# hgpeterson/nuPGCM

Measured on AMD Instinct MI355X. Metric: timesteps/sec (evolve!+invert! loop; inversion SpMV GB/s in 'roofline'), higher is better.
Workload: dtype f64 arithmetic; fp32-STORED Krylov basis and fp32 gather-layout copy of the SpMV input (the library's default at rtol >= 1e-7; products, sums, x += V y and the restart residual are fp64 - the all-fp64 figure is `fp64_basis`); 1 GPU; bowl3D_h0.02: example parameters of examples/bowl_mixing.jl (eps=0.2, alpha=1/2, mu_rho=1, N2=2, BDF2 dt=0.001), full evolve!+invert! timestep loop; tets=526720, nu=2052199, np=98592, nb=707204, nnz_A=126821881, node_block_storage=True, full_nodes=658911, surface_nodes=37733, gmres_memory=20, gmres_itmax=0, initial_guess=x_{n-1} (the reference's warm start), all_solved=True, preconditioner=Diagonal(scalar=73847.66715287707), parallelism=1 GPU

## Files before the change

nupgcm_amd/csrc/gmres.hip:

```cpp
#include <algorithm>
#include <chrono>
#include <cmath>
#include <cstdlib>
#include <type_traits>

#include <hip/hip_ext.h>

#include "common.h"
#include "spmv_device.h"
#include "spmv_window.h"

namespace npg {

constexpr int kKB = 512;
constexpr int kKP = kPartStride;
constexpr int kNS = kKB / kKP;
constexpr int kMaxG = 768;
constexpr int kMaxI = kMaxG / kNS;
constexpr int kNormSlot = kKP - 1;
constexpr int kMaxRows = 2048;

struct Snap {
    double eps, rnorm0, rnorm, beta, zeta;
    int iter, inner, done, npass, first, nreorth, pad0, pad1;
};

struct GParams {
    double atol, rtol, eta2, btol;
    long long itmax;
};

struct GDev {
    CsrDev A;
    const TileDesc *tile_ptr;
    int ntiles, n, mem;
    int nt_int;
    const WTileDesc *wt_ptr;
    WinDev W;
    int nwt, nwt_int, wl;
    int word;
    int wpre;
    int pkind;
    double pscalar;
    const double *pdiag;
    const double *b;
    double *x, *Vi, *w, *wt;
    double *P1, *P2, *PR;
    int G1, G2, GP1, GP2;
    int GR;
    int split;
    int64_t ldv;
    float *Vf;
    int pyth;
    int lazy2;
    int rev;
    GatherMap xg;
    const int32_t *gslot;
    int fast;
    const double *Q1, *Q2, *QR;
    int nQ1, nQ2, nQR;
    Snap *C, *T;
    double *c, *s, *z, *R, *hcol1, *wnorm2;
    double *hist;
    int hist_cap;
    const GParams *prm;
};

__device__ __forceinline__ void sym_givens(double a, double b, double &c, double &s, double &rho) {
    if (b == 0.0) {
        c = (a == 0.0) ? 1.0 : copysign(1.0, a);
        s = 0.0;
        rho = fabs(a);
    } else if (a == 0.0) {
        c = 0.0;
        s = copysign(1.0, b);
        rho = fabs(b);
    } else if (fabs(b) > fabs(a)) {
        const double t = a / b;
        s = copysign(1.0, b) / sqrt(1.0 + t * t);
        c = s * t;
        rho = b / s;
    } else {
        const double t = b / a;
        c = copysign(1.0, a) / sqrt(1.0 + t * t);
        s = c * t;
        rho = a / c;
    }
}

struct KShared {
    double red[kKP];
    double h[kKP], h2[kKP], cc[kKP], ss[kKP], y[kKP];
    Snap T;
    double rho, zcol;
    int fin;
    int reorth;
};

__device__ __forceinline__ void store_partial_row(double acc, double *tmp, double *part) {
    __syncthreads();
    tmp[threadIdx.x] = acc;
    __syncthreads();
    if (threadIdx.x < kKP) {
        double s = 0.0;
#pragma unroll
        for (int sl = 0; sl < kNS; ++sl) s += tmp[sl * kKP + threadIdx.x];
        part[(size_t)blockIdx.x * kKP + threadIdx.x] = s;
    }
}

__device__ void finalize_column(const GDev &d, int colj, KShared &sh, double *tmp) {
    const int t32 = threadIdx.x & (kKP - 1);
    const double h1 = d.hcol1[colj * kKP + t32];
    const double cv = d.c[t32], sv = d.s[t32];
    const Snap prev = d.T[colj];
    const double wnorm2 = d.wnorm2[colj];
    const double q1 = group_sum_dpp<kKP>(t32 <= colj ? h1 * h1 : 0.0);
    const double n2f = wnorm2 - q1;
    const bool need2 = !d.pyth && (!d.lazy2 || !(n2f >= fmax(d.prm->eta2, 1e-4) * wnorm2));
    if (need2) reduce_partials<kNS, kMaxI>(d.Q2, d.nQ2, kKP, tmp, sh.red);
    if (threadIdx.x < kKP) {
        sh.h[threadIdx.x] = h1;
        sh.h2[threadIdx.x] = (need2 && !d.fast && (int)threadIdx.x <= colj) ? sh.red[threadIdx.x] : 0.0;
        sh.cc[threadIdx.x] = cv;
        sh.ss[threadIdx.x] = sv;
    }
    __syncthreads();
    if (threadIdx.x == 0) {
        Snap t = prev;
        sh.fin = (t.done == 0) ? 1 : 0;
        sh.reorth = 0;
        if (t.done == 0) {
            double n2;
            if (d.pyth) {
                n2 = fmax(n2f, 0.0);
                if (n2f < 1e-4 * wnorm2) {
                    t.pad0 += 1;
                    t.done = 5;
                    sh.fin = 0;
                }
            } else if (!need2) {
                n2 = fmax(n2f, 0.0);
            } else {
// ... 84 lines not shown
    double acc = 0.0;
    if (c.done == 0) {
        TileDesc nd = d.tile_ptr[blockIdx.x < (unsigned)d.ntiles ? blockIdx.x : 0];
        for (int t = blockIdx.x; t < d.ntiles; t += gridDim.x) {
            const TileDesc td = nd;
            if (t + (int)gridDim.x < d.ntiles) nd = d.tile_ptr[t + gridDim.x];
            const int r0 = td.r0, r1 = td.r0 + td.nrows;
            spmv_tile<kKB, L, PlainX, kTileNnz, 4, NoProf, false, false, N9>(d.A, PlainX{d.x}, td, tl, sw);
            const int r = threadIdx.x;
            if (r < r1 - r0) {
                const int row = r0 + r;
                const double res = precond_row(d, row) * (d.b[row] - sw[r]);
                d.wt[row] = res;
                if (d.xg.p) d.xg.p[d.xg.pos(row)] = (float)res;
                acc += res * res;
            }
        }
    }
    acc = group_sum_dpp<kKP>(acc);
    store_partial_row((threadIdx.x & (kKP - 1)) == 0 ? acc : 0.0, tmp, d.PR);
}

template <int L, bool FUSED, int XG = 0, bool N9 = false, int WL = 0, bool ORD = true>
__global__ void __launch_bounds__(kKB, FUSED ? 4 : 6) k_gmres_arnoldi(GDev d, int j, int t0, int t1) {
    static_assert(WL == 0 || (XG == 1 && !N9 && !FUSED), "windowed tiles serve the gather-layout instance of the split organisation");
    __shared__ KShared sh;
    __shared__ TileLds tl;
    __shared__ double sw[kTileRows];
    double *tmp = tl.prod;
    using TD = std::conditional_t<WL != 0, WTileDesc, TileDesc>;
    const TD *__restrict__ tiles;
    if constexpr (WL != 0) tiles = d.wt_ptr; else tiles = d.tile_ptr;
    TD nd = tiles[t0 + (int)blockIdx.x < t1 ? t0 + (int)blockIdx.x : 0];
    WinPre pre;
    bool have = false;
    if constexpr (WL != 0) {
        if (d.wpre && t0 + (int)blockIdx.x < t1 && nd.nw) {
            win_first<kKB>(d.W, PaddedX{d.xg}, nd, pre);
            have = true;
        }
    }
    if (j == 0) {
        const Snap c = *d.C;
        reduce_partials<kNS, kMaxI>(d.QR, d.nQR, 1, tmp, sh.red);
        if (threadIdx.x == 0) {
            Snap t = c;
            if (t.done == 0) {
                const double beta = sqrt(sh.red[0]);
                if (t.first) {
                    t.rnorm0 = beta;
                    t.rnorm = beta;
                    t.eps = d.prm->atol + d.prm->rtol * beta;
                    t.first = 0;
                    if (blockIdx.x == 0) d.hist[0] = beta;
                    if (beta == 0.0) t.done = 4;
                }
                t.beta = beta;
                t.zeta = beta;
                t.npass += 1;
            }
            t.inner = 0;
            sh.T = t;
            sh.reorth = 0;
            if (blockIdx.x == 0) d.T[0] = t;
        }
        __syncthreads();
    } else {
        finalize_column(d, j - 1, sh, tmp);
    }
    const Snap T = sh.T;
    if (T.done != 0) return;

    const int k = threadIdx.x & (kKP - 1), slot = threadIdx.x >> 5;
    const double inv_beta = 1.0 / T.beta;
    const bool ro = XG == 0 && sh.reorth != 0;
    const double h2k = (ro && k < j) ? sh.h2[k] : 0.0;
    double acc = 0.0;
    for (int t = t0 + blockIdx.x; t < t1; t += gridDim.x) {
        const TD td = nd;
        if (t + (int)gridDim.x < t1) nd = tiles[t + gridDim.x];
        const int r0 = td.r0, r1 = td.r0 + td.nrows;
        static_assert(kTileRows <= kKB, "one epilogue row per thread");
        double wt_row = 0.0;
        if (!FUSED && (int)threadIdx.x < td.nrows) wt_row = d.wt[td.r0 + threadIdx.x];
        if constexpr (WL != 0) {
            if (td.nw) {
                if (!have) win_first<kKB>(d.W, PaddedX{d.xg}, td, pre);
                have = t + (int)gridDim.x < t1 && nd.nw != 0;
                if (td.r0 < block_rows(d.A))
                    spmv_tile_win<kKB, WL>(d.A, d.W, PaddedX{d.xg}, td, nd, have, pre, tl, sw);
                else
                    spmv_tile_winrows<kKB, L>(d.A, d.W, PaddedX{d.xg}, td, nd, have, pre, tl, sw);
            } else if constexpr (ORD) {
                have = false;
                spmv_tile<kKB, L, PaddedX, kTileNnz, 2, NoProf, false, true, false>(d.A, PaddedX{d.xg}, ordinary(td), tl, sw);
                pre = WinPre{};
            }
        } else if constexpr (XG == 2)
            spmv_tile<kKB, L>(d.A, PaddedX{d.xg}, td, tl, sw);
        else if constexpr (XG == 1)
            spmv_tile<kKB, L, PaddedX, kTileNnz, 2, NoProf, false, true, N9>(d.A, PaddedX{d.xg}, td, tl, sw);
        else
            spmv_tile<kKB, L, CorrectedX, kTileNnz, 4, NoProf, false, false, N9>(
                d.A, CorrectedX{d.wt, d.Vi, sh.h2, ro ? j : 0, d.n, d.ldv, d.Vf}, td, tl, sw);
        const int nr = r1 - r0;
        if (!FUSED) {
            const int r = threadIdx.x;
            if (r < nr) {
                const int row = r0 + r;
                d.w[row] = sw[r] * inv_beta * precond_row(d, row);
                double tv = wt_row;
                if (ro)
                    for (int q = 0; q < j; ++q)
                        tv -= sh.h2[q] * (d.Vf ? (double)d.Vf[vidx(row, q, d.n, d.ldv)] : d.Vi[vidx(row, q, d.n, d.ldv)]);
                if (d.Vf)
                    d.Vf[vidx(row, j, d.n, d.ldv)] = (float)(tv * inv_beta);
                else
                    d.Vi[vidx(row, j, d.n, d.ldv)] = tv * inv_beta;
            }
            continue;
        }
        for (int r = slot; r < nr; r += 2 * kNS) {
            const int rb = r + kNS;
            const bool hb = rb < nr;
            const int rowa = r0 + r, rowb = r0 + (hb ? rb : r);
            double va = (k < j) ? d.Vi[vidx(rowa, k, d.n, d.ldv)] : 0.0;
            double vb = (hb && k < j) ? d.Vi[vidx(rowb, k, d.n, d.ldv)] : 0.0;
            double ta = d.wt[rowa], tb = d.wt[rowb];
            const double wa = sw[r] * inv_beta * precond_row(d, rowa);
            const double wb = hb ? sw[rb] * inv_beta * precond_row(d, rowb) : 0.0;
            if (ro) {
                ta -= group_sum_dpp<kKP>(h2k * va);
                tb -= group_sum_dpp<kKP>(h2k * vb);
            }
            if (k == j) {
                va = ta * inv_beta;
                d.Vi[vidx(rowa, j, d.n, d.ldv)] = va;
                if (hb) {
                    vb = tb * inv_beta;
                    d.Vi[vidx(rowb, j, d.n, d.ldv)] = vb;
                }
            }
            if (k == 0) {
                d.w[rowa] = wa;
                if (hb) d.w[rowb] = wb;
            }
            acc += (k == kNormSlot) ? wa * wa + wb * wb : va * wa + vb * wb;
        }
    }
    if (FUSED) store_partial_row(acc, tmp, d.P1);
}

constexpr int kRB = 256;
constexpr int kMaxRowsI = kMaxG / (kRB / 32);

template <int NG, typename BT>
__device__ __forceinline__ void load_row_cols(const BT *__restrict__ Vi, int64_t row, int64_t ldv, int j,
                                              double (&v)[8 * NG]) {
#pragma unroll
    for (int k = 0; k < 8 * NG; ++k) v[k] = (k <= j) ? (double)Vi[(size_t)k * (size_t)ldv + (size_t)row] : 0.0;
}
template <typename BT>
__device__ __forceinline__ const BT *basis_ptr(const GDev &d);
template <>
__device__ __forceinline__ const double *basis_ptr<double>(const GDev &d) { return d.Vi; }
template <>
__device__ __forceinline__ const float *basis_ptr<float>(const GDev &d) { return d.Vf; }

template <int NG>
__device__ __forceinline__ void store_partial_row_rows(const double (&acc)[8 * NG], double nrm, double *tmp, double *part) {
    const int wave = threadIdx.x >> 6, lane = threadIdx.x & 63;
    __syncthreads();
    if (lane < kKP) tmp[wave * kKP + lane] = 0.0;
    __syncthreads();
#pragma unroll
    for (int k = 0; k < 8 * NG; ++k) {
        const double s = group_sum_dpp<64>(acc[k]);
        if (lane == 0 && k < kNormSlot) tmp[wave * kKP + k] = s;
    }
    const double sn = group_sum_dpp<64>(nrm);
    if (lane == 0) tmp[wave * kKP + kNormSlot] = sn;
    __syncthreads();
    if (threadIdx.x < kKP) {
        double s = 0.0;
#pragma unroll
        for (int w = 0; w < kRB / 64; ++w) s += tmp[w * kKP + threadIdx.x];
        part[(size_t)blockIdx.x * kKP + threadIdx.x] = s;
    }
}

template <int NG>
__device__ __forceinline__ void load_row_pair_cols(const float *__restrict__ Vf, int64_t r0, bool two, int64_t ldv, int j,
                                                   float2 (&v)[8 * NG]) {
#pragma unroll
    for (int k = 0; k < 8 * NG; ++k) {
        float2 f = make_float2(0.f, 0.f);
        if (k <= j) f = *reinterpret_cast<const float2 *>(Vf + (size_t)k * (size_t)ldv + (size_t)r0);
        if (!two) f.y = 0.f;
        v[k] = f;
    }
}
template <int NG>
struct RowPair {
    float2 v[8 * NG];
    double w0, w1;
    int64_t r0;
    bool valid, two;
    __device__ __forceinline__ void load(const GDev &d, int64_t blk, int j) {
        r0 = 2 * (blk * kRB + threadIdx.x);
        valid = r0 < d.n;
        two = r0 + 1 < d.n;
        const int64_t rc = valid ? r0 : 0;
        load_row_pair_cols<NG>(d.Vf, rc, two, d.ldv, j, v);
        const double2 ww = *reinterpret_cast<const double2 *>(d.w + rc);
        w0 = valid ? ww.x : 0.0;
        w1 = (valid && two) ? ww.y : 0.0;
    }
};

template <int NG, typename BT>
__global__ void __launch_bounds__(kRB) k_gmres_dots_rows(GDev d, int j) {
    __shared__ double tmp[(kRB / 64) * kKP];
    double acc[8 * NG];
#pragma unroll
    for (int k = 0; k < 8 * NG; ++k) acc[k] = 0.0;
    double nrm = 0.0;
    if (d.T[j].done == 0) {
        if constexpr (sizeof(BT) == 4) {
            const int64_t nblk = ((int64_t)d.n + 2 * kRB - 1) / (2 * kRB);
            RowPair<NG> cur, nxt;
            int64_t blk = blockIdx.x;
            if (blk < nblk) cur.load(d, blk, j);
            for (; blk < nblk; blk += gridDim.x) {
                const bool more = blk + gridDim.x < nblk;
                if (more) nxt.load(d, blk + gridDim.x, j);
#pragma unroll
                for (int k = 0; k < 8 * NG; ++k) acc[k] += (double)cur.v[k].x * cur.w0 + (double)cur.v[k].y * cur.w1;
                nrm += cur.w0 * cur.w0 + cur.w1 * cur.w1;
                if (more) cur = nxt;
            }
        } else {
            for (int64_t row = blockIdx.x * (int64_t)kRB + threadIdx.x; row < d.n; row += (int64_t)gridDim.x * kRB) {
                double v[8 * NG];
                load_row_cols<NG, BT>(basis_ptr<BT>(d), row, d.ldv, j, v);
                const double wv = d.w[row];
#pragma unroll
                for (int k = 0; k < 8 * NG; ++k) acc[k] += v[k] * wv;
                nrm += wv * wv;
            }
        }
    }
    store_partial_row_rows<NG>(acc, nrm, tmp, d.P1);
}

template <int NG, bool FAST, typename BT>
__global__ void __launch_bounds__(kRB, (NG < 4 || FAST) ? 3 : 2) k_gmres_orth_rows(GDev d, int j) {
    __shared__ double tmp[(kRB / 32) * kKP];
    __shared__ double red[kKP];
    const Snap T = d.T[j];
    constexpr bool kPipe = sizeof(BT) == 4 && FAST;
    const int64_t nblk2 = ((int64_t)d.n + 2 * kRB - 1) / (2 * kRB);
    RowPair<kPipe ? NG : 1> cur;
    if constexpr (kPipe) {
        if (T.done == 0 && (int64_t)blockIdx.x < nblk2) cur.load(d, d.rev ? nblk2 - 1 - blockIdx.x : blockIdx.x, j);
    }
    reduce_partials<kRB / 32, kMaxRowsI>(d.Q1, d.nQ1, kKP, tmp, red);
    double h[8 * NG], acc[8 * NG];
#pragma unroll
    for (int k = 0; k < 8 * NG; ++k) {
        const double hv = (k <= j) ? red[k] : 0.0;
        const unsigned long long b = __double_as_longlong(hv);
        const unsigned lo = __builtin_amdgcn_readfirstlane((unsigned)b), hi = __builtin_amdgcn_readfirstlane((unsigned)(b >> 32));
        h[k] = __longlong_as_double(((unsigned long long)hi << 32) | lo);
        acc[k] = 0.0;
    }
    double nrm = 0.0;
    if (T.done == 0) {
        if (blockIdx.x == 0 && threadIdx.x < kKP) {
            d.hcol1[j * kKP + threadIdx.x] = ((int)threadIdx.x <= j) ? red[threadIdx.x] : 0.0;
            if (threadIdx.x == 0) d.wnorm2[j] = red[kNormSlot];
        }
        if constexpr (kPipe) {
            const int64_t nblk = nblk2;
            RowPair<NG> nxt;
            for (int64_t blk = blockIdx.x; blk < nblk; blk += gridDim.x) {
                const int64_t nb = blk + gridDim.x;
                const bool more = nb < nblk;
                if (more) nxt.load(d, d.rev ? nblk - 1 - nb : nb, j);
                double p0 = cur.w0, p1 = cur.w1;
#pragma unroll
                for (int k = 0; k < 8 * NG; ++k) {
                    p0 -= h[k] * (double)cur.v[k].x;
                    p1 -= h[k] * (double)cur.v[k].y;
                }
                if (cur.valid) {
                    if (cur.two)
                        *reinterpret_cast<double2 *>(d.wt + cur.r0) = make_double2(p0, p1);
                    else
                        d.wt[cur.r0] = p0;
                    if (d.xg.p) {
                        d.xg.p[d.xg.pos((int)cur.r0)] = (float)p0;
                        if (cur.two) d.xg.p[d.xg.pos((int)cur.r0 + 1)] = (float)p1;
                    }
                } else {
                    p0 = 0.0;
                    p1 = 0.0;
                }
                if (!cur.two) p1 = 0.0;
                nrm += p0 * p0 + p1 * p1;
                if (more) cur = nxt;
            }
        } else if constexpr (sizeof(BT) == 4) {
            const int64_t nblk = ((int64_t)d.n + 2 * kRB - 1) / (2 * kRB);
            for (int64_t blk = blockIdx.x; blk < nblk; blk += gridDim.x) {
                const int64_t r0 = 2 * ((d.rev ? nblk - 1 - blk : blk) * kRB + threadIdx.x);
                if (r0 >= d.n) continue;
                const bool two = r0 + 1 < d.n;
                float2 v[8 * NG];
                load_row_pair_cols<NG>(d.Vf, r0, two, d.ldv, j, v);
                const double2 ww = *reinterpret_cast<const double2 *>(d.w + r0);
                double p0 = ww.x, p1 = two ? ww.y : 0.0;
#pragma unroll
                for (int k = 0; k < 8 * NG; ++k) {
                    p0 -= h[k] * (double)v[k].x;
                    p1 -= h[k] * (double)v[k].y;
                }
                if (two)
                    *reinterpret_cast<double2 *>(d.wt + r0) = make_double2(p0, p1);
                else
                    d.wt[r0] = p0;
                if (!FAST) {
#pragma unroll
                    for (int k = 0; k < 8 * NG; ++k) acc[k] += (double)v[k].x * p0 + (double)v[k].y * p1;
                }
                nrm += p0 * p0 + p1 * p1;
            }
        } else {
        const int64_t nblk = ((int64_t)d.n + kRB - 1) / kRB;
        for (int64_t blk = blockIdx.x; blk < nblk; blk += gridDim.x) {
            const int64_t row = (d.rev ? nblk - 1 - blk : blk) * kRB + threadIdx.x;
            if (row >= d.n) continue;
            double v[8 * NG];
            load_row_cols<NG, BT>(basis_ptr<BT>(d), row, d.ldv, j, v);
            double wp = d.w[row];
#pragma unroll
            for (int k = 0; k < 8 * NG; ++k) wp -= h[k] * v[k];
            d.wt[row] = wp;
            if (!FAST) {
#pragma unroll
                for (int k = 0; k < 8 * NG; ++k) acc[k] += v[k] * wp;
            }
            nrm += wp * wp;
        }
        }
    }
    if (!FAST) {
        store_partial_row_rows<NG>(acc, nrm, tmp, d.P2);
    } else {
        const int wave = threadIdx.x >> 6, lane = threadIdx.x & 63;
        const double sn = group_sum_dpp<64>(nrm);
        __syncthreads();
        if (lane == 0) tmp[wave] = sn;
        __syncthreads();
        if (threadIdx.x < kKP) {
            double t = 0.0;
            if (threadIdx.x == kNormSlot)
                for (int w = 0; w < kRB / 64; ++w) t += tmp[w];
            d.P2[(size_t)blockIdx.x * kKP + threadIdx.x] = t;
        }
    }
}

__global__ void __launch_bounds__(kKB, 6) k_gmres_orth(GDev d, int j) {
    __shared__ KShared sh;
    __shared__ double tmp[kNS * kKP];
    const Snap T = d.T[j];
    reduce_partials<kNS, kMaxI>(d.Q1, d.nQ1, kKP, tmp, sh.red);
    if (T.done != 0) return;
    const int k = threadIdx.x & (kKP - 1), slot = threadIdx.x >> 5;
    if (blockIdx.x == 0 && threadIdx.x < kKP) {
        d.hcol1[j * kKP + threadIdx.x] = ((int)threadIdx.x <= j) ? sh.red[threadIdx.x] : 0.0;
        if (threadIdx.x == 0) d.wnorm2[j] = sh.red[kNormSlot];
    }
    const double hk = (k <= j) ? sh.red[k] : 0.0;
    double acc = 0.0;
    const int64_t stride = (int64_t)gridDim.x * kNS;
    for (int64_t row = (int64_t)blockIdx.x * kNS + slot; row < d.n; row += 2 * stride) {
        const int64_t rowb = row + stride;
        const bool hb = rowb < d.n;
        const double va = (k <= j) ? d.Vi[vidx(row, k, d.n, d.ldv)] : 0.0;
        const double vb = (hb && k <= j) ? d.Vi[vidx(rowb, k, d.n, d.ldv)] : 0.0;
        const double wa = d.w[row];
        const double wb = hb ? d.w[rowb] : 0.0;
        const double pa = wa - group_sum_dpp<kKP>(hk * va);
        const double pb = wb - group_sum_dpp<kKP>(hk * vb);
        if (k == 0) {
            d.wt[row] = pa;
            if (hb) d.wt[rowb] = pb;
        }
        acc += (k == kNormSlot) ? pa * pa + pb * pb : va * pa + vb * pb;
    }
    store_partial_row(acc, tmp, d.P2);
}

__global__ void __launch_bounds__(kKB, 6) k_gmres_update(GDev d) {
    __shared__ KShared sh;
    __shared__ double tmp[kNS * kKP];
    __shared__ double Rl[kKP * (kKP + 1) / 2];
    const double zv = d.z[threadIdx.x & (kKP - 1)];
    finalize_column(d, d.mem - 1, sh, tmp);
    const Snap T = sh.T;
    const int kk = T.inner;
    const bool fin = sh.fin != 0;
    const int last = d.mem - 1;
    for (int t = threadIdx.x; t < kk * (kk + 1) / 2; t += kKB) Rl[t] = d.R[t];
    __syncthreads();
    if (fin && threadIdx.x <= (unsigned)last && kk == d.mem)
        Rl[last * (last + 1) / 2 + threadIdx.x] = ((int)threadIdx.x == last) ? sh.rho : sh.h[threadIdx.x];
    __syncthreads();
    if (threadIdx.x < 64) {
        const int lane = threadIdx.x;
        double y = (lane < kk) ? ((fin && lane == last) ? sh.zcol : zv) : 0.0;
        const double btol = d.prm->btol;
        for (int c = kk - 1; c >= 0; --c) {
            const double rcc = Rl[c * (c + 1) / 2 + c];
            double yc = __shfl(y, c, 64);
            yc = (fabs(rcc) <= btol) ? 0.0 : yc / rcc;
            if (lane == c) y = yc;
            if (lane < c) y -= Rl[c * (c + 1) / 2 + lane] * yc;
        }
        if (lane < kKP) sh.y[lane] = (lane < kk) ? y : 0.0;
        if (blockIdx.x == 0 && lane == 0) {
            *d.C = sh.T;
            d.C->inner = 0;
        }
    }
    __syncthreads();
    if (kk == 0) return;
    if (d.ldv && d.Vf) {
        const int64_t nblk = ((int64_t)d.n + 2 * kKB - 1) / (2 * kKB);
        for (int64_t blk = blockIdx.x; blk < nblk; blk += gridDim.x) {
            const int64_t r0 = 2 * (blk * kKB + threadIdx.x);
            if (r0 >= d.n) continue;
            const bool two = r0 + 1 < d.n;
            double2 xx = make_double2(d.x[r0], two ? d.x[r0 + 1] : 0.0);
            for (int q0 = 0; q0 < kk; q0 += 16) {
                float2 f[16];
#pragma unroll
                for (int q = 0; q < 16; ++q) {
                    f[q] = make_float2(0.f, 0.f);
                    if (q0 + q < kk) f[q] = *reinterpret_cast<const float2 *>(d.Vf + (size_t)(q0 + q) * (size_t)d.ldv + (size_t)r0);
                }
// ... 36 lines not shown
        double v[8];
#pragma unroll
        for (int i = 0; i < 8; ++i) {
            const int b = b0 + 32 * i;
            v[i] = b < nrows ? part[(size_t)b * kKP + k] : 0.0;
        }
#pragma unroll
        for (int i = 0; i < 8; ++i) s += v[i];
    }
    tmp[slice * kKP + k] = s;
    __syncthreads();
    if (threadIdx.x < kKP) {
        double t = 0.0;
#pragma unroll
        for (int sl = 0; sl < 32; ++sl) t += tmp[sl * kKP + threadIdx.x];
        out[threadIdx.x] = t;
    }
}

}

using namespace npg;

constexpr int kCfgLen = 17;

struct npg_gmres {
    npg_ctx *ctx = nullptr;
    int64_t n = 0;
    int mem = 20;
    double *Vi = nullptr, *w = nullptr, *wt = nullptr;
    double *P1 = nullptr, *P2 = nullptr, *PR = nullptr;
    Snap *C = nullptr, *T = nullptr;
    double *c = nullptr, *s = nullptr, *z = nullptr, *R = nullptr, *hcol1 = nullptr, *wnorm2 = nullptr;
    double *hist = nullptr;
    int hist_cap = 0;
    GParams *prm = nullptr;
    Snap *h_C = nullptr;
    GParams *h_prm = nullptr;
    int64_t hist_len = 0;
    hipGraph_t graph[2] = {nullptr, nullptr};
    hipGraphExec_t exec[2] = {nullptr, nullptr};
    hipEvent_t ev[2] = {nullptr, nullptr};
    GDev key;
    bool have_graph = false;
    bool profile = false;
    bool explicit_norm = false;
    bool safe_mode = false;
    int split_mode = -1;
    int basis_bits = 0;
    int halo_overlap = -1;
    int dist_graph = -1;
    std::vector<hipEvent_t> pev;
    double prof_ms = 0.0;
    int64_t prof_launches = 0;
    int gather32 = -1;
    float *xg = nullptr;
    int64_t xg_len = 0;
    int xg_key[3] = {-1, -1, -1};
    npg_halo *halo = nullptr;
    double *Rg = nullptr;
    int64_t n_ghost = 0;
    int32_t cfg[kCfgLen] = {};
    bool have_cfg = false;
};

static int fold_rows(npg_gmres *ws, const double *part, int nrows, int slot, hipStream_t st, bool dist) {
    double *out = ws->Rg + slot * kKP;
    if (dist) return fold_allreduce_rows(ws->ctx, part, nrows, out, st);
    hipLaunchKernelGGL(k_reduce_rows, dim3(1), dim3(1024), 0, st, part, nrows, out);
    return NPG_OK;
}

template <int NG, typename BT>
static void launch_rows_bt(const GDev &d, int j, hipStream_t st, bool orth) {
    if (orth && d.fast)
        hipLaunchKernelGGL((k_gmres_orth_rows<NG, true, BT>), dim3(d.GR), dim3(kRB), 0, st, d, j);
    else if (orth)
        hipLaunchKernelGGL((k_gmres_orth_rows<NG, false, BT>), dim3(d.GR), dim3(kRB), 0, st, d, j);
    else
        hipLaunchKernelGGL((k_gmres_dots_rows<NG, BT>), dim3(d.GR), dim3(kRB), 0, st, d, j);
}
template <int NG>
static void launch_rows(const GDev &d, int j, hipStream_t st, bool orth) {
    if (d.Vf)
        launch_rows_bt<NG, float>(d, j, st, orth);
    else
        launch_rows_bt<NG, double>(d, j, st, orth);
}

static void launch_rows_kernel(const GDev &d, int j, hipStream_t st, bool orth) {
    switch ((j + 8) / 8) {
        case 1: launch_rows<1>(d, j, st, orth); break;
        case 2: launch_rows<2>(d, j, st, orth); break;
        case 3: launch_rows<3>(d, j, st, orth); break;
        default: launch_rows<4>(d, j, st, orth); break;
    }
}

template <int L>
static void launch_arnoldi_split(const GDev &d, int grid, int j, int t0, int t1, hipStream_t st, hipEvent_t e0 = nullptr,
                                 hipEvent_t e1 = nullptr) {
    const dim3 g(std::max(1, grid)), b(kKB);
#define NPG_ARNOLDI(...)                                                                          \
    do {                                                                                          \
        if (e0) hipExtLaunchKernelGGL((__VA_ARGS__), g, b, 0, st, e0, e1, 0, d, j, t0, t1);       \
        else hipLaunchKernelGGL((__VA_ARGS__), g, b, 0, st, d, j, t0, t1);                        \
    } while (0)
    if (d.A.pk9) {
        if (d.xg.p)
            NPG_ARNOLDI(k_gmres_arnoldi<L, false, 1, true>);
        else
            NPG_ARNOLDI(k_gmres_arnoldi<L, false, 0, true>);
    } else if (d.xg.p && d.xg.nbr == 0) {
        NPG_ARNOLDI(k_gmres_arnoldi<L, false, 2>);
    } else if (d.xg.p && d.wt_ptr) {
        if (d.wl == 8 && !d.word)
            NPG_ARNOLDI(k_gmres_arnoldi<L, false, 1, false, 8, false>);
        else if (d.wl == 8)
            NPG_ARNOLDI(k_gmres_arnoldi<L, false, 1, false, 8, true>);
        else if (!d.word)
            NPG_ARNOLDI(k_gmres_arnoldi<L, false, 1, false, 4, false>);
        else
            NPG_ARNOLDI(k_gmres_arnoldi<L, false, 1, false, 4, true>);
    } else if (d.xg.p) {
        NPG_ARNOLDI(k_gmres_arnoldi<L, false, 1>);
    } else {
        NPG_ARNOLDI(k_gmres_arnoldi<L, false>);
    }
#undef NPG_ARNOLDI
}
template <int L>
static void launch_residual_L(const GDev &d, hipStream_t st) {
    if (d.A.pk9)
        hipLaunchKernelGGL((k_gmres_residual<L, true>), dim3(d.G1), dim3(kKB), 0, st, d);
    else
        hipLaunchKernelGGL((k_gmres_residual<L>), dim3(d.G1), dim3(kKB), 0, st, d);
}

template <int L>
static int launch_cycle_L(const GDev &d, hipStream_t st, hipEvent_t *pev, npg_gmres *ws, bool dist) {
    int rc = NPG_OK;
    const bool fold = dist;
    static const int overlap_env = getenv("NPG_HALO_OVERLAP") ? atoi(getenv("NPG_HALO_OVERLAP")) : -1;
    const bool kernel_only = dist && comm_is_kernel_only(ws->ctx);
    int want = !dist ? 0 : ws->halo_overlap >= 0 ? ws->halo_overlap : (overlap_env >= 0 ? overlap_env : (kernel_only || ws->ctx->shm ? 1 : 0));
    static const int unverified_ok = getenv("NPG_HALO_OVERLAP_UNVERIFIED") ? atoi(getenv("NPG_HALO_OVERLAP_UNVERIFIED")) : 0;
    if (want && dist && !kernel_only && !ws->ctx->shm && !unverified_ok) {
        static bool told = false;
        if (!told && (told = true))
            fprintf(stderr, "[npg] halo overlap on the RCCL transport was asked for but has never been verified on two physical GPUs: "
                            "running the exchange before the Arnoldi launch instead (NPG_HALO_OVERLAP_UNVERIFIED=1 overrides)\n");
        want = 0;
    }
    const int a_nt = d.wt_ptr ? d.nwt : d.ntiles, a_int = d.wt_ptr ? d.nwt_int : d.nt_int;
    const bool asked = dist && (ws->halo_overlap >= 0 || overlap_env >= 0);
    static const int64_t min_ghosts = getenv("NPG_HALO_OVERLAP_MIN_GHOSTS") ? atoll(getenv("NPG_HALO_OVERLAP_MIN_GHOSTS")) : 200000;
    const bool big = dist && ws->halo && ws->halo->n_ghost >= min_ghosts;
    const bool overlap = dist && d.split && want && a_int > 0 && a_int < a_nt && (asked || (2 * a_int >= a_nt && big));
    const int maxg = ws ? std::min(kMaxG, 3 * ws->ctx->num_cu) : kMaxG;
    static const int reserve_env = getenv("NPG_HALO_RESERVE_CUS") ? atoi(getenv("NPG_HALO_RESERVE_CUS")) : 4;
    const int reserve = std::max(0, std::min(reserve_env, maxg / 6));
    if (dist && getenv("NPG_HALO_OVERLAP_VERBOSE")) {
        static int last = -1;
        const int now = (overlap ? 2 : 0) + (d.split ? 1 : 0);
        if (now != last && (last = now, true))
            fprintf(stderr, "halo overlap %s: %d interior / %d boundary tiles per Arnoldi step (split %d)\n", overlap ? "on" : "off",
                    a_int, a_nt - a_int, d.split);
    }
    float *g32 = (dist && d.xg.p) ? d.xg.p + d.xg.pos(d.n) : nullptr;
    for (int j = 0; j < d.mem; ++j) {
        if (overlap) {
            if ((rc = halo_exchange_async(ws->halo, d.wt, g32, d.gslot, d.xg.p))) return rc;
            if (pev) hipEventRecord(pev[2 * j], st);
            const int gi = kernel_only ? maxg : maxg - 3 * reserve;
            launch_arnoldi_split<L>(d, std::min(a_int, gi), j, 0, a_int, st);
            if ((rc = halo_exchange_wait(ws->halo))) return rc;
            launch_arnoldi_split<L>(d, std::min(a_nt - a_int, maxg), j, a_int, a_nt, st);
            if (pev) hipEventRecord(pev[2 * j + 1], st);
            launch_rows_kernel(d, j, st, false);
        } else {
        if (dist && (rc = halo_exchange_raw(ws->halo, d.wt, g32, d.gslot, d.xg.p))) return rc;
        if (d.split) {
            launch_arnoldi_split<L>(d, std::min(d.G1, std::max(1, a_nt)), j, 0, a_nt, st, pev ? pev[2 * j] : nullptr,
                                    pev ? pev[2 * j + 1] : nullptr);
            launch_rows_kernel(d, j, st, false);
        } else {
            if (pev) hipEventRecord(pev[2 * j], st);
            hipLaunchKernelGGL((k_gmres_arnoldi<L, true>), dim3(d.G1), dim3(kKB), 0, st, d, j, 0, d.ntiles);
            if (pev) hipEventRecord(pev[2 * j + 1], st);
        }
        }
        if (fold && (rc = fold_rows(ws, d.P1, d.GP1, 0, st, dist))) return rc;
        if (d.split)
            launch_rows_kernel(d, j, st, true);
        else
            hipLaunchKernelGGL(k_gmres_orth, dim3(d.G2), dim3(kKB), 0, st, d, j);
        if (fold && !d.pyth && (rc = fold_rows(ws, d.P2, d.GP2, 1, st, dist))) return rc;
    }
    hipLaunchKernelGGL(k_gmres_update, dim3(d.G2), dim3(kKB), 0, st, d);
    if (dist && (rc = halo_exchange_raw(ws->halo, d.x))) return rc;
    launch_residual_L<L>(d, st);
    if (fold && (rc = fold_rows(ws, d.PR, d.G1, 2, st, dist))) return rc;
    return rc;
}

static void launch_residual(const GDev &d, int lanes, hipStream_t st) {
    switch (lanes) {
        case 4: launch_residual_L<4>(d, st); break;
        case 8: launch_residual_L<8>(d, st); break;
        case 16: launch_residual_L<16>(d, st); break;
        default: launch_residual_L<32>(d, st); break;
    }
}

static int launch_cycle(const GDev &d, int lanes, hipStream_t st, hipEvent_t *pev, npg_gmres *ws, bool dist) {
    switch (lanes) {
        case 4: return launch_cycle_L<4>(d, st, pev, ws, dist);
        case 8: return launch_cycle_L<8>(d, st, pev, ws, dist);
        case 16: return launch_cycle_L<16>(d, st, pev, ws, dist);
        default: return launch_cycle_L<32>(d, st, pev, ws, dist);
    }
}

NPG_API int npg_gmres_create(npg_ctx *ctx, int64_t n, int memory, npg_gmres **out) {
    NPG_REQUIRE(ctx && out && n > 0, "npg_gmres_create: bad argument");
    NPG_REQUIRE(memory >= 1 && memory <= kMaxMem, "npg_gmres_create: memory must be in [1,%d]", kMaxMem);
    NPG_REQUIRE(n < INT32_MAX / kKP, "npg_gmres_create: n exceeds the int32 indexing of the interleaved basis");
    npg_gmres *ws = new npg_gmres();
    ws->ctx = ctx;
    ws->n = n;
    ws->mem = memory;
    NPG_HIP(hipSetDevice(ctx->device));
    const size_t vb = ((size_t)n + 2) * sizeof(double);
    const size_t vbytes = ((size_t)n + 32) * sizeof(double) * kKP;
    NPG_HIP(hipMalloc((void **)&ws->Vi, vbytes));
    NPG_HIP(hipMalloc((void **)&ws->w, vb));
    NPG_HIP(hipMalloc((void **)&ws->wt, vb));
    const size_t pb = (size_t)kMaxRows * kKP * sizeof(double);
    NPG_HIP(hipMalloc((void **)&ws->P1, pb));
    NPG_HIP(hipMalloc((void **)&ws->P2, pb));
    NPG_HIP(hipMalloc((void **)&ws->PR, pb));
    NPG_HIP(hipMalloc((void **)&ws->C, sizeof(Snap)));
    NPG_HIP(hipMalloc((void **)&ws->T, sizeof(Snap) * (memory + 1)));
    NPG_HIP(hipMalloc((void **)&ws->c, sizeof(double) * kKP));
    NPG_HIP(hipMalloc((void **)&ws->s, sizeof(double) * kKP));
    NPG_HIP(hipMalloc((void **)&ws->z, sizeof(double) * kKP));
    NPG_HIP(hipMalloc((void **)&ws->R, sizeof(double) * kKP * (kKP + 1) / 2));
    NPG_HIP(hipMalloc((void **)&ws->hcol1, sizeof(double) * kKP * kKP));
    NPG_HIP(hipMalloc((void **)&ws->wnorm2, sizeof(double) * kKP));
    ws->hist_cap = (int)std::min<int64_t>(2 * n + 2, 1 << 22);
    NPG_HIP(hipMalloc((void **)&ws->hist, sizeof(double) * ws->hist_cap));
    NPG_HIP(hipMalloc((void **)&ws->prm, sizeof(GParams)));
    NPG_HIP(hipMalloc((void **)&ws->Rg, 3 * kKP * sizeof(double)));
    NPG_HIP(hipMemsetAsync(ws->Rg, 0, 3 * kKP * sizeof(double), ctx->stream));
    NPG_HIP(hipHostMalloc((void **)&ws->h_C, 2 * sizeof(Snap), hipHostMallocDefault));
    NPG_HIP(hipEventCreateWithFlags(&ws->ev[0], hipEventDisableTiming));
    NPG_HIP(hipEventCreateWithFlags(&ws->ev[1], hipEventDisableTiming));
    NPG_HIP(hipHostMalloc((void **)&ws->h_prm, sizeof(GParams), hipHostMallocDefault));
    NPG_HIP(hipMemsetAsync(ws->Vi, 0, vbytes, ctx->stream));
    NPG_HIP(hipMemsetAsync(ws->w, 0, vb, ctx->stream));
    NPG_HIP(hipMemsetAsync(ws->wt, 0, vb, ctx->stream));
    NPG_HIP(hipMemsetAsync(ws->P1, 0, pb, ctx->stream));
    NPG_HIP(hipMemsetAsync(ws->P2, 0, pb, ctx->stream));
    NPG_HIP(hipMemsetAsync(ws->PR, 0, pb, ctx->stream));
    NPG_HIP(hipMemsetAsync(ws->c, 0, sizeof(double) * kKP, ctx->stream));
    NPG_HIP(hipMemsetAsync(ws->s, 0, sizeof(double) * kKP, ctx->stream));
    NPG_HIP(hipMemsetAsync(ws->z, 0, sizeof(double) * kKP, ctx->stream));
    NPG_HIP(hipMemsetAsync(ws->hcol1, 0, sizeof(double) * kKP * kKP, ctx->stream));
// ... 88 lines not shown
    GDev d;
    memset(&d, 0, sizeof d);
    d.A = csr_view(A);
    d.tile_ptr = A->tile_ptr;
    d.ntiles = A->ntiles;
    d.nt_int = A->ntiles_interior;
    d.n = (int)ws->n;
    d.mem = ws->mem;
    d.pkind = precond_kind;
    d.pscalar = precond_scalar;
    d.pdiag = precond_kind == NPG_PRECOND_DIAG ? precond_diag->d : nullptr;
    d.b = y->d;
    d.x = x->d;
    d.Vi = ws->Vi;
    d.w = ws->w;
    d.wt = ws->wt;
    d.P1 = ws->P1;
    d.P2 = ws->P2;
    d.PR = ws->PR;
    d.G1 = std::max(1, std::min<int>(A->ntiles, std::min(kMaxG, 3 * ctx->num_cu)));
    d.G2 = (int)std::max<int64_t>(1, std::min<int64_t>((ws->n + kNS - 1) / kNS, std::min(kMaxG, 3 * ctx->num_cu)));
    static const int split_env = getenv("NPG_GMRES_SPLIT") ? atoi(getenv("NPG_GMRES_SPLIT")) : -1;
    const int split_req = ws->split_mode >= 0 ? ws->split_mode : split_env;
    d.split = split_req >= 0 ? (split_req != 0) : (ws->n >= 8192 ? 1 : 0);
    if (A->pk9) d.split = 1;
    static const int pyth_env = getenv("NPG_GMRES_PYTH") ? atoi(getenv("NPG_GMRES_PYTH")) : 1;
    d.pyth = (dist && pyth_env && !ws->explicit_norm) ? 1 : 0;
    static const int lazy_env = getenv("NPG_GMRES_LAZY2") ? atoi(getenv("NPG_GMRES_LAZY2")) : 1;
    d.lazy2 = (!dist && lazy_env) ? 1 : 0;
    static const int fast_env = getenv("NPG_GMRES_FAST") ? atoi(getenv("NPG_GMRES_FAST")) : 1;
    d.fast = (d.split && fast_env && reorth_eta <= 0.1 + 1e-12 && (dist || (d.lazy2 && !ws->safe_mode))) ? 1 : 0;
    d.GR = (int)std::max<int64_t>(1, std::min<int64_t>((ws->n + kRB - 1) / kRB, std::min(kMaxG, 3 * ctx->num_cu)));
    if (dist) d.GR = std::min(d.GR, 256);
    static const int rev_env = getenv("NPG_ORTH_REVERSE") ? atoi(getenv("NPG_ORTH_REVERSE")) : 0;
    d.rev = rev_env;
    d.ldv = d.split ? (int64_t)((ws->n + 31) / 32) * 32 : 0;
    static const int basis_env = getenv("NPG_GMRES_BASIS") ? atoi(getenv("NPG_GMRES_BASIS")) : 0;
    const int basis_req = ws->basis_bits ? ws->basis_bits : basis_env;
    const bool basis32 = d.split && (basis_req == 32 || (basis_req == 0 && rtol >= 1e-7));
    d.Vf = basis32 ? reinterpret_cast<float *>(ws->Vi) : nullptr;
    if (basis32) {
        static const int rows_wg = getenv("NPG_GMRES_ROWS_WG") ? std::max(64, atoi(getenv("NPG_GMRES_ROWS_WG"))) : kMaxG;
        d.GR = (int)std::max<int64_t>(1, std::min<int64_t>((ws->n + 2 * kRB - 1) / (2 * kRB), std::min(dist ? 256 : std::min(kMaxG, rows_wg), 3 * ctx->num_cu)));
        d.GP1 = d.GR;
        d.GP2 = d.GR;
    }
    d.GP1 = d.split ? d.GR : d.G1;
    d.GP2 = d.split ? d.GR : d.G2;
    static const int xg_env = getenv("NPG_GMRES_XG") ? atoi(getenv("NPG_GMRES_XG")) : 1;
    d.xg = GatherMap{nullptr, 0, 0, 0, 0};
    static const int xg_csr_env = getenv("NPG_GMRES_XG_CSR") ? atoi(getenv("NPG_GMRES_XG_CSR")) : -1;
    const bool xg_csr = xg_csr_env >= 0 ? xg_csr_env != 0 : ws->n >= 100000;
    if ((ws->gather32 >= 0 ? ws->gather32 : xg_env) && basis32 && d.fast && (A->nnode() > 0 || xg_csr) && (dist ? A->n == A->m + ws->n_ghost : A->n == A->m)) {
        const int64_t nslots = A->wtile_ptr ? gather32_nodes(A) : A->nnode();
        const int64_t nbr = A->block_rows(), need = 4 * nslots + (A->n - nbr) + 8;
        if (ws->xg_len < need) {
            if (ws->xg) NPG_HIP(hipFree(ws->xg));
            ws->xg = nullptr;
            NPG_HIP(hipMalloc((void **)&ws->xg, (size_t)need * sizeof(float)));
            ws->xg_len = need;
            ws->xg_key[0] = -1;
        }
        if (ws->xg_key[0] != A->nfull || ws->xg_key[1] != A->nsurf || ws->xg_key[2] != (int)A->n) {
            NPG_HIP(hipMemsetAsync(ws->xg, 0, (size_t)ws->xg_len * sizeof(float), st));
            ws->xg_key[0] = A->nfull;
            ws->xg_key[1] = A->nsurf;
            ws->xg_key[2] = (int)A->n;
        }
        d.xg = GatherMap{ws->xg, 3 * A->nfull, A->nfull, (int)nbr, (int)(4 * nslots - nbr)};
        d.gslot = A->wtile_ptr ? A->gslot : nullptr;
        static const int win_env = getenv("NPG_GMRES_WINDOW") ? atoi(getenv("NPG_GMRES_WINDOW")) : 1;
        if (win_env && ws->gather32 != 2 && d.split && A->wtile_ptr && !A->pk9 && nbr > 0) {
            d.wt_ptr = A->wtile_ptr;
            d.W = win_view(A);
            d.nwt = A->nwtiles;
            d.nwt_int = A->nwtiles_interior;
            d.wl = A->wlanes;
            static const int ord_env = getenv("NPG_WIN_ORD") ? atoi(getenv("NPG_WIN_ORD")) : 0;
            static const int pre_env = getenv("NPG_WIN_PRE") ? atoi(getenv("NPG_WIN_PRE")) : 1;
            d.word = ord_env || (A->nwrow_tiles == 0 && A->m > A->block_rows());
            d.wpre = pre_env;
        }
    }
    if (dist) {
        d.Q1 = ws->Rg;
        d.Q2 = ws->Rg + kKP;
        d.QR = ws->Rg + 2 * kKP;
        d.nQ1 = d.nQ2 = d.nQR = 1;
    } else {
        d.Q1 = d.P1;
        d.Q2 = d.P2;
        d.QR = d.PR;
        d.nQ1 = d.GP1;
        d.nQ2 = d.GP2;
        d.nQR = d.G1;
    }
    d.C = ws->C;
    d.T = ws->T;
    d.c = ws->c;
    d.s = ws->s;
    d.z = ws->z;
    d.R = ws->R;
    d.hcol1 = ws->hcol1;
    d.wnorm2 = ws->wnorm2;
    d.hist = ws->hist;
    d.hist_cap = ws->hist_cap;
    d.prm = ws->prm;

    if (itmax <= 0) itmax = 2 * ws->n;
    ws->h_prm->atol = atol;
    ws->h_prm->rtol = rtol;
    ws->h_prm->eta2 = reorth_eta <= 0.0 ? -1.0 : reorth_eta * reorth_eta;
    ws->h_prm->btol = std::pow(2.220446049250313e-16, 0.75);
    ws->h_prm->itmax = itmax;
    NPG_HIP(hipMemcpyAsync(ws->prm, ws->h_prm, sizeof(GParams), hipMemcpyHostToDevice, st));
    Snap c0{};
    c0.first = 1;
    ws->h_C[0] = c0;
    NPG_HIP(hipMemcpyAsync(ws->C, ws->h_C, sizeof(Snap), hipMemcpyHostToDevice, st));
    NPG_HIP(hipStreamSynchronize(st));

    static const int traced = getenv("ROCPROFILER_LIBRARY_CTOR") || getenv("ROCPROF_OUTPUT_PATH") || getenv("ROCP_TOOL_LIBRARIES");
    static const int eager = getenv("NPG_GMRES_EAGER") ? atoi(getenv("NPG_GMRES_EAGER")) : traced;
    static bool said = false;
    if (eager && traced && !getenv("NPG_GMRES_EAGER") && !said && (said = true))
        fprintf(stderr, "[npg] rocprofv3 detected: GMRES restart cycles are launched eagerly instead of replayed from hipGraphs "
                        "(rocprofiler-sdk faults on graph launches that wrap the AQL ring; NPG_GMRES_EAGER=0 overrides)\n");
    static const int trace = getenv("NPG_GMRES_TRACE") ? atoi(getenv("NPG_GMRES_TRACE")) : 0;

    static const int dist_graph_env = getenv("NPG_DIST_GRAPH") ? atoi(getenv("NPG_DIST_GRAPH")) : -1;
    const bool kernel_only = dist && comm_is_kernel_only(ws->ctx);
    const bool graph_dist = dist && !ws->ctx->shm &&
                            (kernel_only ? (dist_graph_env != 0 && ws->dist_graph != 0) : ((ws->dist_graph > 0 || dist_graph_env > 0) && ws->ctx->comm));
    auto capture_graphs = [&]() -> int {
        for (int k = 0; k < 2; ++k) {
            if (ws->exec[k]) hipGraphExecDestroy(ws->exec[k]);
            if (ws->graph[k]) hipGraphDestroy(ws->graph[k]);
            ws->exec[k] = nullptr;
            ws->graph[k] = nullptr;
            ws->have_graph = false;
            NPG_HIP(hipStreamBeginCapture(st, hipStreamCaptureModeThreadLocal));
            int rcg = launch_cycle(d, A->lanes, st, nullptr, ws, dist != nullptr);
            if (rcg) {
                hipGraph_t broken = nullptr;
                hipStreamEndCapture(st, &broken);
                if (broken) hipGraphDestroy(broken);
                return rcg;
            }
            NPG_HIP(hipMemcpyAsync(ws->h_C + k, ws->C, sizeof(Snap), hipMemcpyDeviceToHost, st));
            NPG_HIP(hipStreamEndCapture(st, &ws->graph[k]));
            NPG_HIP(hipGraphInstantiate(&ws->exec[k], ws->graph[k], nullptr, nullptr, 0));
        }
        memcpy(&ws->key, &d, sizeof d);
        ws->have_graph = true;
        return NPG_OK;
    };
    const bool use_graph = (!dist || graph_dist) && !eager && !ws->profile;
    if (use_graph && (!ws->have_graph || memcmp(&ws->key, &d, sizeof(GDev)) != 0)) {
        int rcg = capture_graphs();
        if (rcg) return rcg;
    }

    if (dist) {
        int rcd = halo_exchange_raw(ws->halo, d.x);
        if (rcd) return rcd;
    }
    launch_residual(d, A->lanes, st);
    NPG_HIP(hipGetLastError());
    if (dist) {
        int rcd = fold_rows(ws, d.PR, d.G1, 2, st, true);
        if (rcd) return rcd;
    }
    const int64_t max_cycles = (itmax + ws->mem - 1) / ws->mem + 1;
    Snap last{};
    double t_launch = 0.0;
    int64_t n_launch = 0;
    auto enqueue_cycle = [&](int slot) -> int {
        const auto l0 = std::chrono::steady_clock::now();
// ... 176 lines not shown
```

Before: 0.6437 timesteps/s.

## Fold Arnoldi dot partials once and form basis column inside row-dots kernel

Adds a single-block k_gmres_fold_first kernel that reduces the P1 partials once per iteration, writing hcol1 and wnorm2, so the orthogonalization kernel's blocks read one folded row instead of each re-reducing all partials. With the fp32 basis, writing the new basis column v_j = wt/beta moves out of the SpMV epilogue into the row-pair dots kernel, which already streams the rows, removing a separate pass over wt. The orth kernel also returns early when the solve is done. This adds one extra tiny kernel launch per Arnoldi step and changes reduction order slightly.

```diff
diff --git a/nupgcm_amd/csrc/gmres.hip b/nupgcm_amd/csrc/gmres.hip
--- a/nupgcm_amd/csrc/gmres.hip
+++ b/nupgcm_amd/csrc/gmres.hip
@@ -59,6 +59,8 @@
     int fast;
     const double *Q1, *Q2, *QR;
     int nQ1, nQ2, nQR;
+    int onefold;
+    int vdots;
     Snap *C, *T;
     double *c, *s, *z, *R, *hcol1, *wnorm2;
     double *hist;
@@ -309,7 +311,7 @@
         const int r0 = td.r0, r1 = td.r0 + td.nrows;
         static_assert(kTileRows <= kKB, "one epilogue row per thread");
         double wt_row = 0.0;
-        if (!FUSED && (int)threadIdx.x < td.nrows) wt_row = d.wt[td.r0 + threadIdx.x];
+        if (!FUSED && !d.vdots && (int)threadIdx.x < td.nrows) wt_row = d.wt[td.r0 + threadIdx.x];
         if constexpr (WL != 0) {
             if (td.nw) {
                 if (!have) win_first<kKB>(d.W, PaddedX{d.xg}, td, pre);
@@ -336,14 +338,16 @@
             if (r < nr) {
                 const int row = r0 + r;
                 d.w[row] = sw[r] * inv_beta * precond_row(d, row);
-                double tv = wt_row;
-                if (ro)
-                    for (int q = 0; q < j; ++q)
-                        tv -= sh.h2[q] * (d.Vf ? (double)d.Vf[vidx(row, q, d.n, d.ldv)] : d.Vi[vidx(row, q, d.n, d.ldv)]);
-                if (d.Vf)
-                    d.Vf[vidx(row, j, d.n, d.ldv)] = (float)(tv * inv_beta);
-                else
-                    d.Vi[vidx(row, j, d.n, d.ldv)] = tv * inv_beta;
+                if (!d.vdots) {
+                    double tv = wt_row;
+                    if (ro)
+                        for (int q = 0; q < j; ++q)
+                            tv -= sh.h2[q] * (d.Vf ? (double)d.Vf[vidx(row, q, d.n, d.ldv)] : d.Vi[vidx(row, q, d.n, d.ldv)]);
+                    if (d.Vf)
+                        d.Vf[vidx(row, j, d.n, d.ldv)] = (float)(tv * inv_beta);
+                    else
+                        d.Vi[vidx(row, j, d.n, d.ldv)] = tv * inv_beta;
+                }
             }
             continue;
         }
@@ -427,10 +431,11 @@
         v[k] = f;
     }
 }
-template <int NG>
+template <int NG, bool VD = false>
 struct RowPair {
     float2 v[8 * NG];
     double w0, w1;
+    double2 t;
     int64_t r0;
     bool valid, two;
     __device__ __forceinline__ void load(const GDev &d, int64_t blk, int j) {
@@ -438,29 +443,48 @@
         valid = r0 < d.n;
         two = r0 + 1 < d.n;
         const int64_t rc = valid ? r0 : 0;
-        load_row_pair_cols<NG>(d.Vf, rc, two, d.ldv, j, v);
+        load_row_pair_cols<NG>(d.Vf, rc, two, d.ldv, VD ? j - 1 : j, v);
         const double2 ww = *reinterpret_cast<const double2 *>(d.w + rc);
+        if constexpr (VD) t = *reinterpret_cast<const double2 *>(d.wt + rc);
         w0 = valid ? ww.x : 0.0;
         w1 = (valid && two) ? ww.y : 0.0;
     }
 };
 
-template <int NG, typename BT>
+template <int NG, typename BT, bool VD = false>
 __global__ void __launch_bounds__(kRB) k_gmres_dots_rows(GDev d, int j) {
+    static_assert(!VD || sizeof(BT) == 4, "the column is formed by the row-pair kernel of the fp32-stored basis");
     __shared__ double tmp[(kRB / 64) * kKP];
     double acc[8 * NG];
 #pragma unroll
     for (int k = 0; k < 8 * NG; ++k) acc[k] = 0.0;
     double nrm = 0.0;
-    if (d.T[j].done == 0) {
+    const Snap *Tj = d.T + j;
+    if (Tj->done == 0) {
         if constexpr (sizeof(BT) == 4) {
             const int64_t nblk = ((int64_t)d.n + 2 * kRB - 1) / (2 * kRB);
-            RowPair<NG> cur, nxt;
+            RowPair<NG, VD> cur, nxt;
             int64_t blk = blockIdx.x;
             if (blk < nblk) cur.load(d, blk, j);
+            double inv_beta = 0.0;
+            if constexpr (VD) inv_beta = 1.0 / Tj->beta;
             for (; blk < nblk; blk += gridDim.x) {
                 const bool more = blk + gridDim.x < nblk;
                 if (more) nxt.load(d, blk + gridDim.x, j);
+                if constexpr (VD) {
+                    float2 vj = make_float2((float)(cur.t.x * inv_beta), (float)(cur.t.y * inv_beta));
+                    if (cur.valid) {
+                        float *col = d.Vf + (size_t)j * (size_t)d.ldv + (size_t)cur.r0;
+                        if (cur.two)
+                            *reinterpret_cast<float2 *>(col) = vj;
+                        else
+                            *col = vj.x;
+                    }
+                    if (!cur.two) vj.y = 0.f;
+#pragma unroll
+                    for (int k = 0; k < 8 * NG; ++k)
+                        if (k == j) cur.v[k] = vj;
+                }
 #pragma unroll
                 for (int k = 0; k < 8 * NG; ++k) acc[k] += (double)cur.v[k].x * cur.w0 + (double)cur.v[k].y * cur.w1;
                 nrm += cur.w0 * cur.w0 + cur.w1 * cur.w1;
@@ -485,11 +509,15 @@
     __shared__ double tmp[(kRB / 32) * kKP];
     __shared__ double red[kKP];
     const Snap T = d.T[j];
+    if (T.done != 0) {
+        if (threadIdx.x < kKP) d.P2[(size_t)blockIdx.x * kKP + threadIdx.x] = 0.0;
+        return;
+    }
     constexpr bool kPipe = sizeof(BT) == 4 && FAST;
     const int64_t nblk2 = ((int64_t)d.n + 2 * kRB - 1) / (2 * kRB);
     RowPair<kPipe ? NG : 1> cur;
     if constexpr (kPipe) {
-        if (T.done == 0 && (int64_t)blockIdx.x < nblk2) cur.load(d, d.rev ? nblk2 - 1 - blockIdx.x : blockIdx.x, j);
+        if ((int64_t)blockIdx.x < nblk2) cur.load(d, d.rev ? nblk2 - 1 - blockIdx.x : blockIdx.x, j);
     }
     reduce_partials<kRB / 32, kMaxRowsI>(d.Q1, d.nQ1, kKP, tmp, red);
     double h[8 * NG], acc[8 * NG];
@@ -502,84 +530,82 @@
         acc[k] = 0.0;
     }
     double nrm = 0.0;
-    if (T.done == 0) {
-        if (blockIdx.x == 0 && threadIdx.x < kKP) {
-            d.hcol1[j * kKP + threadIdx.x] = ((int)threadIdx.x <= j) ? red[threadIdx.x] : 0.0;
-            if (threadIdx.x == 0) d.wnorm2[j] = red[kNormSlot];
-        }
-        if constexpr (kPipe) {
-            const int64_t nblk = nblk2;
-            RowPair<NG> nxt;
-            for (int64_t blk = blockIdx.x; blk < nblk; blk += gridDim.x) {
-                const int64_t nb = blk + gridDim.x;
-                const bool more = nb < nblk;
-                if (more) nxt.load(d, d.rev ? nblk - 1 - nb : nb, j);
-                double p0 = cur.w0, p1 = cur.w1;
-#pragma unroll
-                for (int k = 0; k < 8 * NG; ++k) {
-                    p0 -= h[k] * (double)cur.v[k].x;
-                    p1 -= h[k] * (double)cur.v[k].y;
+    if (!d.onefold && blockIdx.x == 0 && threadIdx.x < kKP) {
+        d.hcol1[j * kKP + threadIdx.x] = ((int)threadIdx.x <= j) ? red[threadIdx.x] : 0.0;
+        if (threadIdx.x == 0) d.wnorm2[j] = red[kNormSlot];
+    }
+    if constexpr (kPipe) {
+        const int64_t nblk = nblk2;
+        RowPair<NG> nxt;
+        for (int64_t blk = blockIdx.x; blk < nblk; blk += gridDim.x) {
+            const int64_t nb = blk + gridDim.x;
+            const bool more = nb < nblk;
+            if (more) nxt.load(d, d.rev ? nblk - 1 - nb : nb, j);
+            double p0 = cur.w0, p1 = cur.w1;
+#pragma unroll
+            for (int k = 0; k < 8 * NG; ++k) {
+                p0 -= h[k] * (double)cur.v[k].x;
+                p1 -= h[k] * (double)cur.v[k].y;
+            }
+            if (cur.valid) {
+                if (cur.two)
+                    *reinterpret_cast<double2 *>(d.wt + cur.r0) = make_double2(p0, p1);
+                else
+                    d.wt[cur.r0] = p0;
+                if (d.xg.p) {
+                    d.xg.p[d.xg.pos((int)cur.r0)] = (float)p0;
+                    if (cur.two) d.xg.p[d.xg.pos((int)cur.r0 + 1)] = (float)p1;
                 }
-                if (cur.valid) {
-                    if (cur.two)
-                        *reinterpret_cast<double2 *>(d.wt + cur.r0) = make_double2(p0, p1);
-                    else
-                        d.wt[cur.r0] = p0;
-                    if (d.xg.p) {
-                        d.xg.p[d.xg.pos((int)cur.r0)] = (float)p0;
-                        if (cur.two) d.xg.p[d.xg.pos((int)cur.r0 + 1)] = (float)p1;
-                    }
-                } else {
-                    p0 = 0.0;
-                    p1 = 0.0;
-                }
-                if (!cur.two) p1 = 0.0;
-                nrm += p0 * p0 + p1 * p1;
-                if (more) cur = nxt;
-            }
-        } else if constexpr (sizeof(BT) == 4) {
-            const int64_t nblk = ((int64_t)d.n + 2 * kRB - 1) / (2 * kRB);
-            for (int64_t blk = blockIdx.x; blk < nblk; blk += gridDim.x) {
-                const int64_t r0 = 2 * ((d.rev ? nblk - 1 - blk : blk) * kRB + threadIdx.x);
-                if (r0 >= d.n) continue;
-                const bool two = r0 + 1 < d.n;
-                float2 v[8 * NG];
-                load_row_pair_cols<NG>(d.Vf, r0, two, d.ldv, j, v);
-                const double2 ww = *reinterpret_cast<const double2 *>(d.w + r0);
-                double p0 = ww.x, p1 = two ? ww.y : 0.0;
-#pragma unroll
-                for (int k = 0; k < 8 * NG; ++k) {
-                    p0 -= h[k] * (double)v[k].x;
-                    p1 -= h[k] * (double)v[k].y;
-                }
-                if (two)
-                    *reinterpret_cast<double2 *>(d.wt + r0) = make_double2(p0, p1);
-                else
-                    d.wt[r0] = p0;
-                if (!FAST) {
-#pragma unroll
-                    for (int k = 0; k < 8 * NG; ++k) acc[k] += (double)v[k].x * p0 + (double)v[k].y * p1;
-                }
-                nrm += p0 * p0 + p1 * p1;
-            }
-        } else {
-        const int64_t nblk = ((int64_t)d.n + kRB - 1) / kRB;
+            } else {
+                p0 = 0.0;
+                p1 = 0.0;
+            }
+            if (!cur.two) p1 = 0.0;
+            nrm += p0 * p0 + p1 * p1;
+            if (more) cur = nxt;
+        }
+    } else if constexpr (sizeof(BT) == 4) {
+        const int64_t nblk = ((int64_t)d.n + 2 * kRB - 1) / (2 * kRB);
         for (int64_t blk = blockIdx.x; blk < nblk; blk += gridDim.x) {
-            const int64_t row = (d.rev ? nblk - 1 - blk : blk) * kRB + threadIdx.x;
-            if (row >= d.n) continue;
-            double v[8 * NG];
-            load_row_cols<NG, BT>(basis_ptr<BT>(d), row, d.ldv, j, v);
-            double wp = d.w[row];
-#pragma unroll
-            for (int k = 0; k < 8 * NG; ++k) wp -= h[k] * v[k];
-            d.wt[row] = wp;
+            const int64_t r0 = 2 * ((d.rev ? nblk - 1 - blk : blk) * kRB + threadIdx.x);
+            if (r0 >= d.n) continue;
+            const bool two = r0 + 1 < d.n;
+            float2 v[8 * NG];
+            load_row_pair_cols<NG>(d.Vf, r0, two, d.ldv, j, v);
+            const double2 ww = *reinterpret_cast<const double2 *>(d.w + r0);
+            double p0 = ww.x, p1 = two ? ww.y : 0.0;
+#pragma unroll
+            for (int k = 0; k < 8 * NG; ++k) {
+                p0 -= h[k] * (double)v[k].x;
+                p1 -= h[k] * (double)v[k].y;
+            }
+            if (two)
+                *reinterpret_cast<double2 *>(d.wt + r0) = make_double2(p0, p1);
+            else
+                d.wt[r0] = p0;
             if (!FAST) {
 #pragma unroll
-                for (int k = 0; k < 8 * NG; ++k) acc[k] += v[k] * wp;
-            }
-            nrm += wp * wp;
-        }
-        }
+                for (int k = 0; k < 8 * NG; ++k) acc[k] += (double)v[k].x * p0 + (double)v[k].y * p1;
+            }
+            nrm += p0 * p0 + p1 * p1;
+        }
+    } else {
+    const int64_t nblk = ((int64_t)d.n + kRB - 1) / kRB;
+    for (int64_t blk = blockIdx.x; blk < nblk; blk += gridDim.x) {
+        const int64_t row = (d.rev ? nblk - 1 - blk : blk) * kRB + threadIdx.x;
+        if (row >= d.n) continue;
+        double v[8 * NG];
+        load_row_cols<NG, BT>(basis_ptr<BT>(d), row, d.ldv, j, v);
+        double wp = d.w[row];
+#pragma unroll
+        for (int k = 0; k < 8 * NG; ++k) wp -= h[k] * v[k];
+        d.wt[row] = wp;
+        if (!FAST) {
+#pragma unroll
+            for (int k = 0; k < 8 * NG; ++k) acc[k] += v[k] * wp;
+        }
+        nrm += wp * wp;
+    }
     }
     if (!FAST) {
         store_partial_row_rows<NG>(acc, nrm, tmp, d.P2);
@@ -595,6 +621,33 @@
                 for (int w = 0; w < kRB / 64; ++w) t += tmp[w];
             d.P2[(size_t)blockIdx.x * kKP + threadIdx.x] = t;
         }
+    }
+}
+
+__global__ void __launch_bounds__(kRB) k_gmres_fold_first(GDev d, int j, double *out) {
+    constexpr int NS = kRB / 32;
+    __shared__ double tmp[NS * kKP];
+    const int done = d.T[j].done;
+    const int k = threadIdx.x & (kKP - 1), slice = threadIdx.x >> 5;
+    const int nrows = d.GP1;
+    double v[kMaxRowsI];
+#pragma unroll
+    for (int i = 0; i < kMaxRowsI; ++i) {
+        const int b = slice + NS * i;
+        v[i] = d.P1[(size_t)(b < nrows ? b : 0) * kKP + k];
+    }
+    double s = 0.0;
+#pragma unroll
+    for (int i = 0; i < kMaxRowsI; ++i) s += (slice + NS * i < nrows) ? v[i] : 0.0;
+    tmp[slice * kKP + k] = s;
+    __syncthreads();
+    if (threadIdx.x < kKP && done == 0) {
+        double t = 0.0;
+#pragma unroll
+        for (int sl = 0; sl < NS; ++sl) t += tmp[sl * kKP + threadIdx.x];
+        out[threadIdx.x] = t;
+        d.hcol1[j * kKP + threadIdx.x] = ((int)threadIdx.x <= j) ? t : 0.0;
+        if (threadIdx.x == kNormSlot) d.wnorm2[j] = t;
     }
 }
 
@@ -797,7 +850,9 @@
 }
 template <int NG>
 static void launch_rows(const GDev &d, int j, hipStream_t st, bool orth) {
-    if (d.Vf)
+    if (d.Vf && d.vdots && !orth)
+        hipLaunchKernelGGL((k_gmres_dots_rows<NG, float, true>), dim3(d.GR), dim3(kRB), 0, st, d, j);
+    else if (d.Vf)
         launch_rows_bt<NG, float>(d, j, st, orth);
     else
         launch_rows_bt<NG, double>(d, j, st, orth);
@@ -899,6 +954,7 @@
             launch_arnoldi_split<L>(d, std::min(d.G1, std::max(1, a_nt)), j, 0, a_nt, st, pev ? pev[2 * j] : nullptr,
                                     pev ? pev[2 * j + 1] : nullptr);
             launch_rows_kernel(d, j, st, false);
+            if (d.onefold) hipLaunchKernelGGL(k_gmres_fold_first, dim3(1), dim3(kRB), 0, st, d, j, const_cast<double *>(d.Q1));
         } else {
             if (pev) hipEventRecord(pev[2 * j], st);
             hipLaunchKernelGGL((k_gmres_arnoldi<L, true>), dim3(d.G1), dim3(kKB), 0, st, d, j, 0, d.ntiles);
@@ -1153,6 +1209,9 @@
             d.wpre = pre_env;
         }
     }
+    const char *onefold_env = getenv("NPG_GMRES_ONEFOLD");
+    d.onefold = (!dist && d.split && d.fast && !(onefold_env && atoi(onefold_env) == 0)) ? 1 : 0;
+    d.vdots = (d.onefold && d.Vf) ? 1 : 0;
     if (dist) {
         d.Q1 = ws->Rg;
         d.Q2 = ws->Rg + kKP;
@@ -1165,6 +1224,10 @@
         d.nQ1 = d.GP1;
         d.nQ2 = d.GP2;
         d.nQR = d.G1;
+        if (d.onefold) {
+            d.Q1 = ws->Rg;
+            d.nQ1 = 1;
+        }
     }
     d.C = ws->C;
     d.T = ws->T;
```

After: 0.6603 timesteps/s, median of 6. +2.6%, better.
